# Rinoahu/pangenome

Hardware: AMD Instinct MI355X
Metric: Gbp/s k-mer->rdBG build at k=27; bit-exact region table vs numba ref (higher is better)
Workload: dtype u8; 1 GPU; C3: 100 x 5 Mbp variants (0.1% SNP, 0.01% indel), two alternating batches of the same population (genomes 0-99, 100-199); k=27, strands=-c 2 (dBG both strands), bases_per_gpu=500000568, fasta_bytes_per_gpu=508334450, parallelism=single GPU

## Files before the change

### pangenome_amd/csrc/pg_abi.hip

```cpp
#include <chrono>
#include <cstring>
#include <string>

#include "../../include/pangenome.h"
#include "pg_internal.h"
#include "pg_text.h"

struct pg_ctx {
  pg::Ctx c;
};

static thread_local std::string g_err;

template <class F>
static int guard(F&& f) {
  try {
    f();
    return PG_OK;
  } catch (const pg::Error& e) {
    g_err = e.what();
    return e.code;
  } catch (const std::bad_alloc&) {
    g_err = "out of host memory";
    return PG_ENOMEM;
// ... 45 lines not shown
    PG_HIP(hipStreamCreateWithFlags(&x->c.stream3, hipStreamNonBlocking));
    {
      int lo = 0, hi = 0;
      PG_HIP(hipDeviceGetStreamPriorityRange(&lo, &hi));
      PG_HIP(hipStreamCreateWithPriority(&x->c.stream_hi, hipStreamNonBlocking, hi));
    }
    for (auto& e : x->c.ev) PG_HIP(hipEventCreateWithFlags(&e, hipEventDisableTiming));
    for (auto& e : x->c.cev) PG_HIP(hipEventCreateWithFlags(&e, hipEventDisableTiming));
    PG_HIP(hipEventCreateWithFlags(&x->c.rec_ev, hipEventDisableTiming));
    PG_HIP(hipEventCreateWithFlags(&x->c.ext_ev, hipEventDisableTiming));
    PG_HIP(hipDeviceGetAttribute(&x->c.n_cu, hipDeviceAttributeMultiprocessorCount, device));
    *out = x;
  });
}

void pg_destroy(pg_ctx* x) {
  if (!x) return;
  pg::Ctx& c = x->c;
  (void)hipSetDevice(c.device);
  (void)hipStreamSynchronize(c.stream);
  pg::DevBuf* bufs[] = {&c.fasta_own, &c.span_sum, &c.span_start, &c.n_sel, &c.rec_start, &c.rec_len,
                        &c.rec_hdr, &c.rec_ptr, &c.rec_flag, &c.cls, &c.p2, &c.e16, &c.scratch, &c.table, &c.ovf, &c.flags,
                        &c.recA_key, &c.recA_mw, &c.ctrA, &c.recS_key[0], &c.recS_key[1], &c.recS_mw[0],
                        &c.recS_mw[1], &c.ctrS, &c.snapA, &c.rseg, &c.k5_ctr, &c.tile_sched, &c.tile_desc, &c.k3_queue,
                        &c.k3_hint, &c.part_cnt, &c.tile_cnt, &c.tile_off, &c.occ, &c.edge_tab, &c.pair_tab,
                        &c.edge_out, &c.edge_exp, &c.lab_tab, &c.lab_list, &c.rows_buf, &c.xyz_off,
                        &c.text_buf, &c.clu_text, &c.mk_mat, &c.fr_tab, &c.fr_spec, &c.fr_grp, &c.fr_text,
                        &c.cmp_shared, &c.cmp_curve, &c.nj_dist, &c.rg_nodes, &c.rg_links, &c.rg_paths, &c.rg_steps, &c.rg_text,
                        &c.rs_tab, &c.rs_blob, &c.preload,
                        &c.dump_cnt};
  for (auto* b : bufs) b->release();
  pg::pool_destroy(c);
  c.stage_pin.release();
  c.rec_pack.release();
  c.h_pin.release();
  c.h_out.release();
  c.tile_pin.release();
  for (auto& b : c.dump_pin) b.release();
  c.t0.destroy();
  c.t1.destroy();
  c.t6.destroy();
  c.t_rs.destroy();
  c.t_nj.destroy();
  for (auto& t : c.t_bt) t.destroy();
  for (auto& e : c.ev)
    if (e) (void)hipEventDestroy(e);
  for (auto e : c.cev)
// ... 1365 lines not shown
```

### pangenome_amd/csrc/pg_dbg.hip

```cpp
#include <algorithm>
#include <type_traits>
#include <cstdio>
#include <cstdlib>
#include <cstring>

#include <rocprim/rocprim.hpp>

#include "pg_internal.h"

#ifndef PG_EXP_BITS
#define PG_EXP_BITS 0
#endif

namespace pg {

#ifdef PG_DEBUG_BOUNDS
__device__ unsigned long long g_dbg[16 + 16 * 4 * 5];
__device__ __forceinline__ bool pg_bok(bool ok, unsigned code, long long a, long long b) {
  if (!ok) {
    const unsigned slot = code % 16;
    const unsigned long long i = atomicAdd(&g_dbg[slot], 1ull);
    if (i < 4) {
      unsigned long long* e = g_dbg + 16 + (slot * 4 + i) * 5;
      e[0] = code; e[1] = (unsigned long long)a; e[2] = (unsigned long long)b; e[3] = blockIdx.x; e[4] = threadIdx.x;
// ... 427 lines not shown
  }
  return covered;
}

struct Stage {
  long long qt, a0, hi, plo, phi, ra0, rend;
};
__device__ __forceinline__ void ref_span(Stage& g, int k, long long rfs, long long rfn) {
  g.plo = g.qt - 1 - DRIFT > 0 ? g.qt - 1 - DRIFT : 0;
  g.phi = g.qt + TILE + k + 1 + DRIFT < rfn ? g.qt + TILE + k + 1 + DRIFT : rfn;
  g.ra0 = (rfs + g.plo) & ~15ll;
  g.rend = rfs + g.phi;
}
__device__ __forceinline__ Stage stage_of(const TileDesc& td, int k, bool dedup, long long rfs, long long rfn) {
  Stage g;
  g.qt = (long long)td.stripe * TILE;
  const long long lo = td.rs + (g.qt >= 2 ? g.qt - 2 : 0);
  g.hi = td.rs + (g.qt + TILE + k + 2 < td.rn ? g.qt + TILE + k + 2 : td.rn);
  g.a0 = lo & ~15ll;
  g.plo = g.phi = g.ra0 = g.rend = 0;
  if (dedup) ref_span(g, k, rfs, rfn);
  return g;
}

__host__ __device__ __forceinline__ void xcd_chunk(uint64_t ntiles, uint32_t b0, uint32_t b1, uint32_t bt, uint64_t x,
                                                   uint64_t& t, uint64_t& te) {
  const uint64_t xs = ntiles * x / 8, xl = ntiles * (x + 1) / 8 - xs;
  t = xs + xl * b0 / bt;
  te = xs + xl * b1 / bt;
}

#ifdef PG_COVER_LEGACY
__global__ void __launch_bounds__(CBLOCK)
k_cover(const uint8_t* __restrict__ cls, const TileDesc* __restrict__ descs, WorkItem* __restrict__ queue,
        unsigned long long* __restrict__ qcount, unsigned long long qcap, int k, int ref, long long rfs,
        long long rfn, int ref2, long long r2s, long long r2n, int* __restrict__ hints, int nrec,
        uint64_t ngroups, uint32_t b0, uint32_t b1, uint32_t bt) {
  __shared__ __attribute__((aligned(16))) uint8_t s_cls[QM][SPAN + 16];
  __shared__ __attribute__((aligned(16))) uint8_t s_ref[2][RSPAN];
  __shared__ unsigned s_best[QM][2][NANCH];
  __shared__ uint32_t s_scan[CBLOCK / 64];
  __shared__ unsigned long long s_qbase;
  __shared__ MemGeo s_geo[QM];
  __shared__ Drifts s_dr[QM][2];
  uint64_t g, ge;
  xcd_chunk(ngroups, b0, b1, bt, blockIdx.x & 7, g, ge);
// ... 390 lines not shown
          const int s = 4 * (3 * ri + j);
          const uint32_t nz = ((w0 >> s) & 15u) | ((w1 >> s) & 15u) << 4 | ((w2 >> s) & 15u) << 8;
          covered |= ((rel >= lo) & (rel <= hi)) ? map_cover(nz, sh, k) : 0u;
        }
      }
    }
    cov[m] = covered;
    const bool work = ((live >> m) & 1u) && q0 <= last && covered != (1u << IW) - 1u;
    wmask |= (uint32_t)work << m;
    nwk += work ? 1u : 0u;
  }
  uint32_t nwork;
  uint32_t pos = block_excl_scan<CBLOCK>(nwk, s_scan, nwork);
  const unsigned sub = blockIdx.x % NQ;
  if (t == 0) s_qbase = nwork ? atomicAdd(qcount + QSTRIDE * sub, (unsigned long long)nwork) : 0ull;
  __syncthreads();
#pragma unroll
  for (int m = 0; m < QM; ++m)
    if ((wmask >> m) & 1u) queue[sub * qcap + s_qbase + pos++] = WorkItem{mrs[m], mrn[m] - k, q0, cov[m], 0u};
}

#endif

struct TriGeo {
  int ibhi, lo, hi, lo1, hi1;
};

constexpr int RPADW = 4;
constexpr int RSTAGEW = (RSPAN + 15) / 16 + 2;
constexpr int RDW = (RPADW + RSTAGEW + 16 + 3) / 4 * 4;
constexpr int LW = 7;
static_assert(IW * 4 == 64 && CBLOCK == 64 * QM, "a lane owns 4 segments; a wave owns a member");
#ifndef PG_HWIN2P
#define PG_HWIN2P 56
#endif
constexpr int HWIN2P = PG_HWIN2P;
constexpr int NAP_DEFAULT = 4;
template <int NAP>
constexpr int astep_p() { return (TILE - ALEN - 16) / (NAP - 1); }

template <int NAP>
struct Drifts2 {
  int n;
  int U[NAP], lo[NAP], hi[NAP];
  int d[NAP];
};
__device__ __forceinline__ uint32_t p2_word(const uint32_t* p2, long long i, uint64_t n_p2) {
  return (i >= 0 && (uint64_t)i < n_p2) ? p2[i] : 0u;
}
// ... 77 lines not shown
  }
  auto take = [&](auto W) {
    constexpr int w = decltype(W)::value;
#pragma unroll
    for (int i = 0; i < 8; ++i) out[i] = raw[w + i];
  };
  switch (__builtin_amdgcn_readfirstlane(idx & 3)) {
    case 0: take(std::integral_constant<int, 0>{}); break;
    case 1: take(std::integral_constant<int, 1>{}); break;
    case 2: take(std::integral_constant<int, 2>{}); break;
    default: take(std::integral_constant<int, 3>{}); break;
  }
}
__device__ __forceinline__ uint32_t even_bits(uint32_t x) {
  x = (x | (x >> 1)) & 0x33333333u;
  x = (x | (x >> 2)) & 0x0F0F0F0Fu;
  x = (x | (x >> 4)) & 0x00FF00FFu;
  return (x | (x >> 8)) & 0x0000FFFFu;
}

template <int NAP>
__global__ void __launch_bounds__(CBLOCK, 8)
k_cover_p(const uint32_t* __restrict__ p2, const uint8_t* __restrict__ e16, uint64_t n_p2,
          const uint8_t* __restrict__ cls_dbg, const TileDesc* __restrict__ descs, WorkItem* __restrict__ queue, unsigned long long* __restrict__ qcount,
          unsigned long long qcap, int k, int ref, long long rfs, long long rfn, int ref2, long long r2s,
          long long r2n, int* __restrict__ hints, int nrec, uint64_t ngroups, uint32_t b0, uint32_t b1, uint32_t bt) {
  static_assert(NAP >= 2 && QM * NAP + QM * 2 * NAP <= CBLOCK, "anchor loads and triple geometry: one thread each");
  constexpr int ASTEPP = astep_p<NAP>();
  __shared__ __attribute__((aligned(16))) uint32_t s_ref[2][RDW];
  __shared__ uint32_t s_anc[QM][NAP][2];
  __shared__ unsigned s_best[QM][2][NAP];
  __shared__ uint32_t s_scan[CBLOCK / 64];
  __shared__ unsigned long long s_qbase;
  __shared__ Drifts2<NAP> s_dr[QM][2];
  __shared__ TriGeo s_tri[QM * 2 * NAP];
  __shared__ uint32_t s_rexc;
  uint64_t g, ge;
  xcd_chunk(ngroups, b0, b1, bt, blockIdx.x & 7, g, ge);
  g += blockIdx.x >> 3;
  if (g >= ge) return;
  const int t = (int)threadIdx.x;
  const long long qt = (long long)descs[QM * g].stripe * TILE;
  RefGeo rg[2];
  long long rd0[2];
  int rnw[2];
#pragma unroll
  for (int ri = 0; ri < 2; ++ri) {
    const long long s = ri ? r2s : rfs, n = ri ? r2n : rfn;
    rg[ri].plo = qt - 1 - DRIFT > 0 ? qt - 1 - DRIFT : 0;
    rg[ri].phi = qt + TILE + k + 1 + DRIFT < n ? qt + TILE + k + 1 + DRIFT : n;
    rg[ri].rfn = n;
    rd0[ri] = (s + rg[ri].plo) >> 4;
    rnw[ri] = (int)(((s + rg[ri].phi + 15) >> 4) - rd0[ri]);
    rg[ri].rbase = 16 * RPADW + s - 16 * rd0[ri];
  }
  long long mrs[QM], mrn[QM];
  uint32_t dm0 = 0, dm1 = 0, live = 0;
#pragma unroll
  for (int m = 0; m < QM; ++m) {
    const TileDesc td = descs[QM * g + m];
    mrs[m] = td.rs;
    mrn[m] = td.rn;
    const bool d0 = td.r >= 0 && ref >= 0 && ref != td.r;
    live |= (uint32_t)(td.r >= 0) << m;
    dm0 |= (uint32_t)d0 << m;
    dm1 |= (uint32_t)(d0 && ref2 >= 0 && ref2 != td.r) << m;
  }
  const int mw = __builtin_amdgcn_readfirstlane(t >> 6), lw = t & 63;
  uint32_t M[LW], eex = 0;
  {
    long long rsm = mrs[0];
#pragma unroll
    for (int y = 1; y < QM; ++y) if (mw == y) rsm = mrs[y];
    const long long wb = ((rsm + qt - 1) >> 4) + 4 * lw, a = wb & ~3ll;
    const bool on = (dm0 >> mw) & 1u;
#pragma unroll
    for (int i = 0; i < LW; ++i) M[i] = on ? p2_word(p2, wb + i, n_p2) : 0u;
#pragma unroll
    for (int i = 0; i < 3; ++i)
      if (on && a + 4 * i >= 0 && (uint64_t)(a + 4 * i + 4) <= n_p2 + 16)
        eex |= *reinterpret_cast<const uint32_t*>(e16 + a + 4 * i);
  }
  if (t == 0) s_rexc = 0u;
  if (t < QM * NAP) {
    const int m = t / NAP, ai = t % NAP;
    long long rs = mrs[0];
#pragma unroll
    for (int y = 1; y < QM; ++y) rs = m == y ? mrs[y] : rs;
    const long long ga = rs + qt + 8 + (long long)ai * ASTEPP, x = ga >> 4;
    const uint32_t sb = 2u * (uint32_t)(ga & 15);
    uint32_t P0 = 0, P1 = 0, P2 = 0;
    if ((dm0 >> m) & 1u) { P0 = p2_word(p2, x, n_p2); P1 = p2_word(p2, x + 1, n_p2); P2 = p2_word(p2, x + 2, n_p2); }
    s_anc[m][ai][0] = __builtin_amdgcn_alignbit(P1, P0, sb);
    s_anc[m][ai][1] = __builtin_amdgcn_alignbit(P2, P1, sb);
  } else if (t >= CBLOCK - QM * 2 * NAP) {
    const int x = t - (CBLOCK - QM * 2 * NAP), m = x / (2 * NAP), ri = (x / NAP) & 1, ai = x % NAP;
    (&s_best[0][0][0])[x] = ~0u;
    TriGeo G{0, 0, -1, 0, -1};
    if ((((ri ? dm1 : dm0) >> m) & 1u)) {
      const TileDesc td = descs[QM * g + m];
      const int hh = hints[(size_t)(blockIdx.x & 7) * 2 * nrec + (ri ? nrec : 0) + td.r];
      const int h = hh < 0 ? DRIFT : hh;
      const RefGeo& R = ri ? rg[1] : rg[0];
      const long long a = qt + 8 + (long long)ai * ASTEPP;
      G.ibhi = (int)(R.rbase + a + DRIFT);
      G.lo = max(G.ibhi - 2 * DRIFT, (int)(R.rbase + R.plo));
      G.hi = a + ALEN > td.rn ? -1 : min(G.ibhi, (int)(R.rbase + R.phi) - ALEN);
      G.lo1 = max(G.lo, G.ibhi - (h + HWIN2P));
      G.hi1 = min(G.hi, G.ibhi - (h - HWIN2P));
    }
    s_tri[x] = G;
  }
  cover_barrier();
  {
    static_assert(RSTAGEW <= 2 * CBLOCK, "two words per thread and reference");
    uint32_t v[2][2], ex = 0;
#pragma unroll
    for (int ri = 0; ri < 2; ++ri) {
      const int nw = (ri ? dm1 != 0 : dm0 != 0) ? rnw[ri] : 0;
#pragma unroll
      for (int h = 0; h < 2; ++h) {
        const int i = t + h * CBLOCK;
        v[ri][h] = i < nw ? p2_word(p2, rd0[ri] + i, n_p2) : 0u;
        if (i < nw && PG_BOK(rd0[ri] + i >= 0 && (uint64_t)(rd0[ri] + i) < n_p2, 12, rd0[ri] + i, n_p2) &&
            e16[rd0[ri] + i])
          ex |= 1u << ri;
      }
    }
#pragma unroll
    for (int ri = 0; ri < 2; ++ri)
#pragma unroll
      for (int h = 0; h < 2; ++h)
        if (t + h * CBLOCK < rnw[ri] && PG_BOK(RPADW + t + h * CBLOCK < RDW, 13, rnw[ri], t))
          s_ref[ri][RPADW + t + h * CBLOCK] = v[ri][h];
    if (ex) atomicOr(&s_rexc, ex);
  }
  cover_barrier();
  {
    const uint32_t rexc = s_rexc;
    if (rexc & 1u) dm0 = dm1 = 0u;
    if (rexc & 2u) dm1 = 0u;
  }
  if (dm0) cover_search_p(s_anc, s_ref, s_tri, s_best, dm0, dm1);
  if (t < QM * 2 * NAP) {
    const int m = t / (2 * NAP), ri = (t / NAP) & 1, ai = t % NAP;
    if ((((ri ? dm1 : dm0) >> m) & 1u)) {
      const unsigned* B = s_best[m][ri];
      const unsigned b = B[ai];
      auto first = [&](int j) {
        if (B[j] == ~0u) return false;
        for (int i = 0; i < j; ++i)
          if ((B[i] & 0xFFFFu) == (B[j] & 0xFFFFu)) return false;
        return true;
      };
      int slot = 0;
      for (int j = 0; j < ai; ++j) slot += first(j) ? 1 : 0;
      const bool keep = first(ai);
      bool last = b != ~0u;
      for (int j = ai + 1; j < NAP; ++j) last &= B[j] == ~0u;
      long long rs = mrs[0];
#pragma unroll
      for (int y = 1; y < QM; ++y) rs = m == y ? mrs[y] : rs;
      const int r = descs[QM * g + m].r;
      (void)PG_BOK(r >= 0 && r < nrec, 52, (long long)r, (long long)nrec);
      if (last) hints[(size_t)(blockIdx.x & 7) * 2 * nrec + (ri ? nrec : 0) + r] = (int)(b & 0xFFFFu);
      Drifts2<NAP>& D = s_dr[m][ri];
      if (keep) {
        const RefGeo R = ri ? rg[1] : rg[0];
        const long long pos16 = 16 * ((rs + qt - 1) >> 4) - rs;
        const int d = (int)(b & 0xFFFFu) - DRIFT;
        const long long pl = R.plo + 1 > 1 ? R.plo + 1 : 1;
        const long long ph = R.rfn - k - IW < R.phi - IW - k ? R.rfn - k - IW : R.phi - IW - k;
        const long long lo = pl + d - qt, hi = ph + d - qt;
        D.U[slot] = (int)(R.rbase + pos16 - d);
        D.lo[slot] = (int)(lo < -(1ll << 30) ? -(1ll << 30) : lo);
        D.hi[slot] = (int)(hi > (1ll << 30) ? (1ll << 30) : hi);
        D.d[slot] = d;
      }
      if (ai == NAP - 1) D.n = slot + (keep ? 1 : 0);
    }
  }
  cover_barrier();
  const int m = __builtin_amdgcn_readfirstlane(t >> 6), l = t & 63;
  long long rs = mrs[0], rn = mrn[0];
#pragma unroll
  for (int y = 1; y < QM; ++y) if (m == y) { rs = mrs[y]; rn = mrn[y]; }
  const long long last = rn - k;
  uint32_t covS[4] = {0u, 0u, 0u, 0u};
  bool mex = false;
  if ((dm0 >> m) & 1u) {
    const long long p0 = rs + qt - 1, wb = (p0 >> 4) + 4 * l;
    const int sh2 = 2 * (int)(p0 & 15);
    (void)PG_BOK(wb + LW <= (long long)n_p2 + 4 || wb > (long long)n_p2, 11, wb, n_p2);
    (void)wb;
    mex = eex != 0u;
    const int L = k + 2;
    const int P = L >= 16 ? 16 : L >= 8 ? 8 : L >= 4 ? 4 : 2;
    const uint32_t rsh = 2u * (uint32_t)(L - P);
#pragma unroll
    for (int ri = 0; ri < 2; ++ri) {
      if (ri && !((dm1 >> m) & 1u)) break;
      const int nd = __builtin_amdgcn_readfirstlane(s_dr[m][ri].n);
#pragma unroll 1
      for (int j = 0; j < nd; ++j) {
        const int U = __builtin_amdgcn_readfirstlane(s_dr[m][ri].U[j]);
        const int lo = __builtin_amdgcn_readfirstlane(s_dr[m][ri].lo[j]);
        const int hi = __builtin_amdgcn_readfirstlane(s_dr[m][ri].hi[j]);
        int iw = (U >> 4) + 4 * l;
        if (iw < 0 || iw + 12 > RDW) iw &= 3;
        if (!PG_BOK(iw >= 0 && iw + 12 <= RDW, 14, iw, U)) iw = 0;
        uint32_t raw[12];
        {
          const uint4* r16 = reinterpret_cast<const uint4*>(s_ref[ri]);
#pragma unroll
          for (int q = 0; q < 3; ++q) {
            uint4 v = r16[(iw >> 2) + q];
            asm volatile("" : "+v"(v.x), "+v"(v.y), "+v"(v.z), "+v"(v.w));
            raw[4 * q] = v.x; raw[4 * q + 1] = v.y; raw[4 * q + 2] = v.z; raw[4 * q + 3] = v.w;
// ... 32 lines not shown
          covS[s] |= (rel >= lo && rel <= hi) ? ~S & 0x55555555u : 0u;
#ifdef PG_DEBUG_BOUNDS
          {
            const long long q0 = qt + rel;
            const int dd = __builtin_amdgcn_readfirstlane(s_dr[m][ri].d[j]);
            const long long fs = ri ? r2s : rfs;
            const uint32_t cvd = (rel >= lo && rel <= hi && q0 > 0 && q0 + IW <= last) ? (~S & 0x55555555u) : 0u;
            for (int i = 0; i < 16; ++i)
              if ((cvd >> (2 * i)) & 1u) {
                const long long q = q0 + i;
                bool eq = true;
                for (int x = -1; x <= k; ++x) eq &= cls_dbg[rs + q + x] == cls_dbg[fs + q - dd + x];
                (void)pg_bok(eq, 31, (long long)q, (long long)dd);
              }
          }
#endif
        }
      }
    }
  }
  uint32_t nwk = 0, wmask = 0, cov[4];
#pragma unroll
  for (int s = 0; s < 4; ++s) {
    const long long q0 = qt + 64 * l + 16 * s;
    const bool interior = q0 > 0 && q0 + IW <= last;
    cov[s] = interior && !mex ? even_bits(covS[s]) : 0u;
    const bool work = ((live >> m) & 1u) && q0 <= last && cov[s] != (1u << IW) - 1u;
    wmask |= (uint32_t)work << s;
    nwk += work ? 1u : 0u;
  }
  uint32_t nwork;
  uint32_t pos = block_excl_scan<CBLOCK>(nwk, s_scan, nwork);
  const unsigned sub = blockIdx.x % NQ;
  if (t == 0) {
    s_qbase = nwork ? atomicAdd(qcount + QSTRIDE * sub, (unsigned long long)nwork) : 0ull;
    (void)PG_BOK(nwork <= QM * CBLOCK && s_qbase + nwork <= qcap, 42, (long long)nwork, (long long)s_qbase);
  }
  cover_barrier();
#pragma unroll
  for (int s = 0; s < 4; ++s)
    if ((wmask >> s) & 1u) {
      if (PG_BOK(s_qbase + pos < qcap && rs >= 0 && qt + 64 * l + 16 * s <= rn, 15, s_qbase + pos, rs))
        queue[sub * qcap + s_qbase + pos] = WorkItem{rs, rn - k, qt + 64 * l + 16 * s, cov[s], 0u};
      ++pos;
    }
}

template <typename... A>
static void launch_cover_p(int na, dim3 grid, hipStream_t s, A... a) {
  switch (na) {
    case 3: hipLaunchKernelGGL(k_cover_p<3>, grid, dim3(CBLOCK), 0, s, a...); break;
    case 4: hipLaunchKernelGGL(k_cover_p<4>, grid, dim3(CBLOCK), 0, s, a...); break;
    case 5: hipLaunchKernelGGL(k_cover_p<5>, grid, dim3(CBLOCK), 0, s, a...); break;
    case 6: hipLaunchKernelGGL(k_cover_p<6>, grid, dim3(CBLOCK), 0, s, a...); break;
    default: hipLaunchKernelGGL(k_cover_p<8>, grid, dim3(CBLOCK), 0, s, a...); break;
  }
}

#ifdef PG_DEBUG_BOUNDS
__global__ void k_dbg_counters(const unsigned long long* __restrict__ qcount, unsigned long long lim, unsigned code,
                               unsigned chunk) {
  const unsigned sub = threadIdx.x;
  if (sub < NQ) {
    const unsigned long long v = qcount[QSTRIDE * sub];
    (void)pg_bok(v <= lim, code, (long long)v, (long long)(chunk * 1000 + sub));
  }
// ... 687 lines not shown
    b += __shfl_down(b, o, 64);
    m += __shfl_down(m, o, 64);
  }
  if ((threadIdx.x & 63) == 0) {
    s_red[0][threadIdx.x >> 6] = a;
    s_red[1][threadIdx.x >> 6] = b;
    s_red[2][threadIdx.x >> 6] = m;
  }
  __syncthreads();
  if (threadIdx.x == 0) {
    unsigned long long sa = 0, sb = 0, sm = 0;
    for (int w = 0; w < RB_T / 64; ++w) { sa += s_red[0][w]; sb += s_red[1][w]; sm += s_red[2][w]; }
    unsigned long long* o = R.ctr + (uint64_t)blockIdx.x * RB_CTR;
    o[0] = sa;
    o[1] = sb;
    if constexpr (KEYS) o[2] = s_mcur;
    else o[2] = sm;
  }
}

constexpr uint32_t LEAD = 4;
__global__ void k_tiles(const uint32_t* __restrict__ sched, uint32_t nj, uint32_t lead_stripes, uint32_t lead_off,
                        const long long* __restrict__ rec_start, const long long* __restrict__ rec_len,
                        TileDesc* __restrict__ out, uint64_t ngroups) {
  const uint32_t* off = sched;
  const uint32_t* nf = sched + nj + 1;
  const uint32_t* ord = nf + nj;
  for (uint64_t t = blockIdx.x * (uint64_t)blockDim.x + threadIdx.x; t < ngroups * QM;
       t += (uint64_t)gridDim.x * blockDim.x) {
    const uint64_t g = t / QM;
    const uint32_t m = (uint32_t)(t % QM);
    uint32_t lo = 0, hi = nj;
    while (hi - lo > 1) {
      const uint32_t mid = (lo + hi) >> 1;
      if (off[mid] <= g) lo = mid; else hi = mid;
    }
    uint32_t i = (uint32_t)(g - off[lo]);
    const bool lead = lo < lead_stripes;
    int r = -1, stripe;
    if (lead && i == 0) {
      stripe = (int)lo;
      if (m == 0) r = (int)ord[0];
    } else {
      if (lead) --i;
      stripe = (int)(lo - lead_off);
      const uint32_t f = i * QM + m;
      if (f < nf[lo]) r = (int)ord[1 + f];
    }
    out[t] = r >= 0 ? TileDesc{rec_start[r], rec_len[r], r, stripe, 0} : TileDesc{0, 0, -1, stripe, 0};
  }
}

constexpr int EXE = 8;
__global__ void __launch_bounds__(256) k_export_dbg(TableView T, uint64_t nw, uint64_t ntot, int k,
                                                   unsigned long long* __restrict__ keys,
                                                   unsigned short* __restrict__ masks, uint64_t cap,
                                                   unsigned long long* __restrict__ counter) {
  __shared__ uint32_t s_scan[4];
  __shared__ unsigned long long s_base;
  for (uint64_t c0 = blockIdx.x * (uint64_t)(256 * EXE); c0 < ntot; c0 += (uint64_t)gridDim.x * 256 * EXE) {
    uint32_t m[EXE];
    uint32_t cnt = 0;
#pragma unroll
    for (int e = 0; e < EXE; ++e) {
      const uint64_t i = c0 + (uint64_t)threadIdx.x * EXE + e;
      m[e] = i < ntot ? entry_mask(T, nw, i) : 0u;
      cnt += ((m[e] & PRES_A) ? 1u : 0u) + ((m[e] & PRES_B) ? 1u : 0u);
    }
    uint32_t tot;
    const uint32_t pre = block_excl_scan<256>(cnt, s_scan, tot);
    if (threadIdx.x == 0) s_base = tot ? atomicAdd(counter, (unsigned long long)tot) : 0ull;
    __syncthreads();
// ... 211 lines not shown
  const uint32_t lead_off = follow ? 0u : LEAD;
  const uint32_t nj = nt.empty() ? 0u : (uint32_t)(follow ? nt[0].first : lead_s + LEAD);
  const size_t skip = follow ? 0 : 1;
  std::vector<uint32_t> sched(2 * nj + 2 + nt.size());
  uint64_t total = 0;
  size_t live = nt.size();
  for (uint32_t j = 0; j < nj; ++j) {
    sched[j] = (uint32_t)total;
    uint64_t cnt = j < lead_s ? 1 : 0, nfol = 0;
    if (j >= lead_off) {
      const uint64_t jf = j - lead_off;
      while (live && nt[live - 1].first <= jf) --live;
      nfol = live > skip ? live - skip : 0;
      cnt += (nfol + QM - 1) / QM;
    }
    sched[nj + 1 + j] = (uint32_t)nfol;
    total += cnt;
  }
  sched[nj] = (uint32_t)total;
  if (follow) sched[2 * nj + 1] = 0u;
  for (size_t i = 0; i < nt.size(); ++i) sched[2 * nj + 1 + (follow ? 1 : 0) + i] = (uint32_t)nt[i].second;
  if (total * QM >= (1ull << 32)) throw Error(-22, "make_tiles: too many tiles");
  c.tile_desc.reserve(sizeof(TileDesc) * (QM * total + 1));
  if (total) {
    c.tile_pin.reserve(4 * sched.size());
    c.tile_sched.reserve(4 * sched.size());
    std::memcpy(c.tile_pin.p, sched.data(), 4 * sched.size());
    PG_HIP(hipMemcpyAsync(c.tile_sched.p, c.tile_pin.p, 4 * sched.size(), hipMemcpyHostToDevice, st));
    hipLaunchKernelGGL(k_tiles, dim3(grid_for(QM * total, 256, 2048)), dim3(256), 0, st,
                       c.tile_sched.as<uint32_t>(), nj, (uint32_t)lead_s, lead_off, c.rec_start.as<long long>(),
                       c.rec_len.as<long long>(), c.tile_desc.as<TileDesc>(), total);
    PG_HIP(hipGetLastError());
  }
  if (follow) {
    c.tile_sig_len.clear();
  } else {
    c.tile_sig_len = c.h_rec_len;
    c.tile_sig_flag = flag;
    c.tile_k = c.k;
  }
  c.n_tiles = total;
  return total;
}

static BinOut stageA_begin(Ctx& c, uint64_t cap, FillList& fl, bool reset = true) {
  if (reset) {
    c.capA = cap;
    c.recA_key.reserve(8 * NREG * cap);
    c.recA_mw.reserve(4 * NREG * cap);
    c.ctrA.reserve(8 * CSTRIDE * NREG);
    c.flags.reserve(4 * N_FLAGS + 16 * MCHK);
    fl.add(c.ctrA.p, 8 * CSTRIDE * NREG);
    fl.add(c.flags.p, 4 * N_FLAGS + 16 * MCHK);
  }
// ... 269 lines not shown
  if (!c.n_records) return;
  hipLaunchKernelGGL(k_short_emit, dim3(grid_for(c.n_records, IBLOCK, 1024)), dim3(IBLOCK), 0, s, packed_cls(c),
                     c.rec_start.as<long long>(), c.rec_len.as<long long>(), c.rec_flag.as<uint8_t>(), c.n_records,
                     c.k, shift, rc0, c.tv, O);
  PG_HIP(hipGetLastError());
}

enum { SA_WHOLE = 0, SA_FIRST = 1, SA_MORE = 2, SA_TAIL = 3, SA_FIRST_TAIL = 4, SA_MORE_TAIL = 5 };
static void enqueue_stageA(Ctx& c, uint64_t cap, uint64_t ntiles, int rc0, int extra_empty, int part = SA_WHOLE,
                           bool join = true) {
  const uint64_t shift = pow5(c.k - 1);
  hipStream_t s0 = c.stream, s1 = c.stream2;
  FillList fl;
  const bool begin = part == SA_WHOLE || part == SA_FIRST || part == SA_FIRST_TAIL;
  const bool tail = part == SA_WHOLE || part == SA_TAIL || part == SA_FIRST_TAIL || part == SA_MORE_TAIL;
  const BinOut O = stageA_begin(c, cap, fl, begin);
  if (part == SA_TAIL) ntiles = 0;
#ifdef PG_COVER_LEGACY
  if (c.k3_cover == 1 || c.k3_cover == 2) ensure_cls(c);
#endif
#ifdef PG_DEBUG_BOUNDS
  ensure_cls(c);
#endif
  const uint8_t* cls = c.cls.as<uint8_t>();
  const PackedCls pc = packed_cls(c);
  const dim3 b(IBLOCK);
  int nch = ntiles >= (uint64_t)K3_CHUNKS * K3_CHUNK_MIN ? K3_CHUNKS : 1;
  if (c.k3_chunks > 0) nch = std::min(6, c.k3_chunks);
  if (!ntiles) nch = 0;
  const uint32_t tailw = c.k3_tail ? (uint32_t)c.k3_tail : 10u;
  const uint32_t headw = c.k3_head ? (uint32_t)c.k3_head : 16u;
  uint32_t cb[8] = {};
  for (int i = 1; i <= nch; ++i) cb[i] = cb[i - 1] + (i == nch ? tailw : i == 1 ? headw : 16u);
  const uint32_t cbt = nch ? cb[nch] : 1u;
  uint64_t gc[8] = {}, qoff[8] = {}, qcapc[8] = {}, items = 0;
  for (int i = 0; i < nch; ++i) {
    for (int x = 0; x < 8; ++x) {
      uint64_t t, te;
      xcd_chunk(ntiles, cb[i], cb[i + 1], cbt, (uint64_t)x, t, te);
      gc[i] = std::max<uint64_t>(gc[i], 8 * (te - t));
    }
    qcapc[i] = (gc[i] + NQ - 1) / NQ * (QM * CBLOCK);
    qoff[i] = items;
    items += NQ * qcapc[i];
  }
  const size_t qbytes = sizeof(WorkItem) * items, cbytes = 8 * QSTRIDE * NQ;
  if (nch) {
    c.k3_queue.reserve(qbytes + cbytes * nch);
    fl.add(c.k3_queue.as<uint8_t>() + qbytes, cbytes * nch);
    fl.add(c.k3_hint.p, 16 * 4 * (c.n_records + 1), 0xFFFFFFFFu);
  }
  const bool side = part == SA_WHOLE;
  if (side) {
    fl.launch(s1);
    PG_HIP(hipEventRecord(c.ev[0], s1));
    PG_HIP(hipStreamWaitEvent(s0, c.ev[0], 0));
  }
  c.t1.init();
  c.t1.start(s0);
  if (!side) fl.launch(s0);
#ifdef PG_DEBUG_BOUNDS
  for (int i = 0; i < nch; ++i)
    hipLaunchKernelGGL(k_dbg_counters, dim3(1), dim3(64), 0, s0,
                       reinterpret_cast<const unsigned long long*>(c.k3_queue.as<uint8_t>() + qbytes) + (cbytes / 8) * i,
                       0ull, 41u, (unsigned)i);
#endif
  const unsigned wgrid = (unsigned)c.n_cu * (c.k3_wblk & 15 ? c.k3_wblk & 15 : K3_WBLK);
  const unsigned wgrid_last = c.k3_wblk >> 4 ? (unsigned)c.n_cu * (c.k3_wblk >> 4) : wgrid;
  auto* q = c.k3_queue.as<WorkItem>();
  auto* qn = reinterpret_cast<unsigned long long*>(c.k3_queue.as<uint8_t>() + qbytes);
  const long long rfs = c.k3_ref >= 0 ? c.h_rec_start[c.k3_ref] : 0, rfn = c.k3_ref >= 0 ? c.h_rec_len[c.k3_ref] : 0;
  const long long r2s = c.k3_ref2 >= 0 ? c.h_rec_start[c.k3_ref2] : 0;
  const long long r2n = c.k3_ref2 >= 0 ? c.h_rec_len[c.k3_ref2] : 0;
  const TileDesc* td = c.tile_desc.as<TileDesc>();
  bool short_done = false;
  if (!side) {
    PG_HIP(hipEventRecord(c.ev[0], s0));
    PG_HIP(hipStreamWaitEvent(s1, c.ev[0], 0));
  }
  for (int i = 0; i < nch; ++i) {
    auto* qi = q + qoff[i];
    auto* qni = qn + (cbytes / 8) * i;
#ifdef PG_COVER_LEGACY
    if (gc[i] && c.k3_cover == 1)
      hipLaunchKernelGGL(k_cover, dim3((unsigned)gc[i]), dim3(CBLOCK), 0, s0, cls, td, qi, qni, (unsigned long long)qcapc[i],
                         c.k, c.k3_ref, rfs, rfn, c.k3_ref2, r2s, r2n, c.k3_hint.as<int>(), (int)c.n_records, ntiles,
                         cb[i], cb[i + 1], cbt);
    else if (gc[i] && c.k3_cover == 2)
      hipLaunchKernelGGL(k_cover_q, dim3((unsigned)gc[i]), dim3(CBLOCK), 0, s0, cls, (uint64_t)c.cls.cap, td, qi, qni,
                         (unsigned long long)qcapc[i], c.k, c.k3_ref, rfs, rfn, c.k3_ref2, r2s, r2n,
                         c.k3_hint.as<int>(), (int)c.n_records, ntiles, cb[i], cb[i + 1], cbt);
    else
#endif
    if (gc[i])
      launch_cover_p(c.k3_anchors ? c.k3_anchors : NAP_DEFAULT, dim3((unsigned)gc[i]), s0, c.p2.as<uint32_t>(),
                     c.e16.as<uint8_t>(), (uint64_t)(c.p2.cap / 4), cls, td, qi, qni, (unsigned long long)qcapc[i], c.k,
                     c.k3_ref, rfs, rfn, c.k3_ref2, r2s, r2n, c.k3_hint.as<int>(), (int)c.n_records, ntiles,
                     cb[i], cb[i + 1], cbt);
    PG_HIP(hipGetLastError());
#ifdef PG_DEBUG_BOUNDS
    for (int j = 0; j < nch; ++j)
      hipLaunchKernelGGL(k_dbg_counters, dim3(1), dim3(64), 0, s0, qn + (cbytes / 8) * j,
                         j <= i ? (unsigned long long)qcapc[j] : 0ull, j <= i ? 43u : 44u, (unsigned)(i * 10 + j));
#endif
    hipStream_t ws = s1;
    if (nch > 1 && i + 1 == nch) {
      ws = s0;
      if (tail) {
        launch_short(c, s1, rc0, shift, O);
        short_done = true;
      }
    } else {
      PG_HIP(hipEventRecord(c.ev[1 + i], s0));
      PG_HIP(hipStreamWaitEvent(s1, c.ev[1 + i], 0));
    }
    const uint64_t mi = std::min<uint64_t>(NQ * qcapc[i], c.windows_fw / IW + c.n_records + 1);
    const unsigned gw = nch > 1 ? (i + 1 == nch ? wgrid_last : wgrid) : grid_for(mi, IBLOCK, 16384);
    const bool halves = c.k3_emit != 1;
    auto* kw = rc0 ? (halves ? k_emit_work<true, 2> : k_emit_work<true, 1>)
                   : (halves ? k_emit_work<false, 2> : k_emit_work<false, 1>);
    hipLaunchKernelGGL(kw, dim3(gw), b, 0, ws, pc, qi, qni, (unsigned long long)qcapc[i], c.k, shift, c.tv, O);
// ... 581 lines not shown
```

### pangenome_amd/csrc/pg_internal.h

```cpp
#pragma once
#include <hip/hip_runtime.h>

#include <algorithm>
#include <atomic>
#include <chrono>
#include <cstdint>
#include <cstdlib>
#include <cstring>
#include <stdexcept>
#include <string>
#include <functional>
#include <vector>

#include "pg_common.h"

namespace pg {

struct Error : std::runtime_error {
  int code;
  Error(int c, const std::string& m) : std::runtime_error(m), code(c) {}
};

#define PG_HIP(x)                                                                       \
  do {                                                                                  \
// ... 197 lines not shown
  DevBuf k5_ctr;
  uint64_t rseg_cap = 0, rseg_nseg = 0;
  std::vector<uint64_t> rseg_cnt;
  uint64_t n_records_a = 0;
  double u_ratio = 0, r_ratio = 0;

  DevBuf tile_sched;
  PinBuf tile_pin;
  uint64_t n_tiles = 0;
  int tile_k = 0;
  int k3_ref = -1;
  int k3_ref2 = -1;
  DevBuf part_cnt;
  uint64_t part_counts[64] = {};
  uint64_t part_sums[64] = {};
  uint64_t merge_sum = 0, merge_rows = 0;
  uint64_t work_items = 0;
  uint64_t part_total = 0;
  int part_nparts = 0;
  uint64_t part_gen = ~0ull;
  uint64_t build_gen = 0;
  DevBuf k3_hint;
  DevBuf tile_desc;
  DevBuf k3_queue;
  std::vector<int64_t> tile_sig_len;
  std::vector<uint8_t> tile_sig_flag;

  DevBuf tile_cnt, tile_off;
  DevBuf occ;
  DevBuf edge_tab, pair_tab;
  DevBuf edge_out;
  DevBuf edge_exp;
  uint64_t edge_cap = 0, pair_cap = 0, n_edges = 0;
  bool edges_ready = false;
  DevBuf lab_tab;
  uint64_t lab_cap = 0;
  DevBuf lab_list;
  uint64_t n_labels = 0;
  DevBuf rows_buf;
  uint64_t n_rows = 0;
  bool rows_ready = false;
  DevBuf xyz_off;
  uint64_t xyz_total = 0;
  bool xyz_sized = false;
  DevBuf text_buf;
  DevBuf clu_text;
// ... 388 lines not shown
```

Before: 443.8 Gbp/s.

## Precompute per-group cover geometry in k_tiles and hoist reference loads in k_cover_p

k_tiles now also writes a 16-byte-aligned GroupGeo record per tile group, holding the stripe offset, member/dedup bitmasks, per-member word bases, shifts and relative bounds, and per-reference span parameters. k_cover_p reads this record instead of recomputing it from TileDesc entries and 64-bit reference arithmetic. The per-XCD chunk bounds are now computed on the host and passed as a kernel argument, and the reference-word loads are issued before the first barrier rather than after it. The aim is to cut scalar and divergent setup work and to overlap the global loads in the cover kernel. The cost is an extra device buffer, a heavier k_tiles kernel, and values clamped to 30 bits, which relies on relative offsets staying within that range.

Result: no change. 452.8 Gbp/s, median of 6 (+2.0%).

```diff
diff --git a/pangenome_amd/csrc/pg_abi.hip b/pangenome_amd/csrc/pg_abi.hip
--- a/pangenome_amd/csrc/pg_abi.hip
+++ b/pangenome_amd/csrc/pg_abi.hip
@@ -91,7 +91,7 @@
   pg::DevBuf* bufs[] = {&c.fasta_own, &c.span_sum, &c.span_start, &c.n_sel, &c.rec_start, &c.rec_len,
                         &c.rec_hdr, &c.rec_ptr, &c.rec_flag, &c.cls, &c.p2, &c.e16, &c.scratch, &c.table, &c.ovf, &c.flags,
                         &c.recA_key, &c.recA_mw, &c.ctrA, &c.recS_key[0], &c.recS_key[1], &c.recS_mw[0],
-                        &c.recS_mw[1], &c.ctrS, &c.snapA, &c.rseg, &c.k5_ctr, &c.tile_sched, &c.tile_desc, &c.k3_queue,
+                        &c.recS_mw[1], &c.ctrS, &c.snapA, &c.rseg, &c.k5_ctr, &c.tile_sched, &c.tile_desc, &c.tile_geo, &c.k3_queue,
                         &c.k3_hint, &c.part_cnt, &c.tile_cnt, &c.tile_off, &c.occ, &c.edge_tab, &c.pair_tab,
                         &c.edge_out, &c.edge_exp, &c.lab_tab, &c.lab_list, &c.rows_buf, &c.xyz_off,
                         &c.text_buf, &c.clu_text, &c.mk_mat, &c.fr_tab, &c.fr_spec, &c.fr_grp, &c.fr_text,
diff --git a/pangenome_amd/csrc/pg_dbg.hip b/pangenome_amd/csrc/pg_dbg.hip
--- a/pangenome_amd/csrc/pg_dbg.hip
+++ b/pangenome_amd/csrc/pg_dbg.hip
@@ -473,6 +473,10 @@
   if (dedup) ref_span(g, k, rfs, rfn);
   return g;
 }
+
+struct TriGeo {
+  int ibhi, lo, hi, lo1, hi1;
+};
 
 __host__ __device__ __forceinline__ void xcd_chunk(uint64_t ntiles, uint32_t b0, uint32_t b1, uint32_t bt, uint64_t x,
                                                    uint64_t& t, uint64_t& te) {
@@ -909,9 +913,41 @@
 
 #endif
 
-struct TriGeo {
-  int ibhi, lo, hi, lo1, hi1;
+struct RefSpan {
+  long long rd0;
+  int rnw;
+  int ph;
+  int ibhi0, lomin, himax;
+  int pl;
 };
+struct MemberGeo {
+  long long rs, last;
+  long long wb;
+  int r;
+  int sh2;
+  int lastrel;
+  int arel;
+  int U0[2];
+};
+struct alignas(16) GroupGeo {
+  long long qt;
+  uint32_t bits;
+  uint32_t pad;
+  RefSpan ref[2];
+  MemberGeo mem[QM];
+};
+static_assert(QM <= 8 && sizeof(RefSpan) == 32 && sizeof(MemberGeo) == 48 && sizeof(GroupGeo) == 16 + 64 + 48 * QM &&
+                  sizeof(GroupGeo) % 16 == 0,
+              "wide aligned loads of a header, a reference or a member");
+struct HintGeo {
+  int r, U0, pl, ph;
+};
+struct XcdBounds {
+  uint32_t g0[8], ge[8];
+};
+__host__ __device__ __forceinline__ int clamp30(long long v) {
+  return (int)(v < -(1ll << 30) ? -(1ll << 30) : v > (1ll << 30) ? (1ll << 30) : v);
+}
 
 constexpr int RPADW = 4;
 constexpr int RSTAGEW = (RSPAN + 15) / 16 + 2;
@@ -1035,9 +1071,11 @@
 template <int NAP>
 __global__ void __launch_bounds__(CBLOCK, 8)
 k_cover_p(const uint32_t* __restrict__ p2, const uint8_t* __restrict__ e16, uint64_t n_p2,
-          const uint8_t* __restrict__ cls_dbg, const TileDesc* __restrict__ descs, WorkItem* __restrict__ queue, unsigned long long* __restrict__ qcount,
-          unsigned long long qcap, int k, int ref, long long rfs, long long rfn, int ref2, long long r2s,
-          long long r2n, int* __restrict__ hints, int nrec, uint64_t ngroups, uint32_t b0, uint32_t b1, uint32_t bt) {
+#ifdef PG_DEBUG_BOUNDS
+          const uint8_t* __restrict__ cls_dbg, long long rfs, long long r2s,
+#endif
+          const GroupGeo* __restrict__ geo, WorkItem* __restrict__ queue, unsigned long long* __restrict__ qcount,
+          unsigned long long qcap, int k, int* __restrict__ hints, int nrec, XcdBounds xb) {
   static_assert(NAP >= 2 && QM * NAP + QM * 2 * NAP <= CBLOCK, "anchor loads and triple geometry: one thread each");
   constexpr int ASTEPP = astep_p<NAP>();
   __shared__ __attribute__((aligned(16))) uint32_t s_ref[2][RDW];
@@ -1047,60 +1085,47 @@
   __shared__ unsigned long long s_qbase;
   __shared__ Drifts2<NAP> s_dr[QM][2];
   __shared__ TriGeo s_tri[QM * 2 * NAP];
+  __shared__ HintGeo s_hg[QM * 2 * NAP];
   __shared__ uint32_t s_rexc;
-  uint64_t g, ge;
-  xcd_chunk(ngroups, b0, b1, bt, blockIdx.x & 7, g, ge);
-  g += blockIdx.x >> 3;
-  if (g >= ge) return;
+  const uint32_t xcd = blockIdx.x & 7;
+  const uint32_t g = xb.g0[xcd] + (blockIdx.x >> 3);
+  if (g >= xb.ge[xcd]) return;
   const int t = (int)threadIdx.x;
-  const long long qt = (long long)descs[QM * g].stripe * TILE;
-  RefGeo rg[2];
-  long long rd0[2];
-  int rnw[2];
+  const GroupGeo& G = geo[g];
+  const int mw = __builtin_amdgcn_readfirstlane(t >> 6), lw = t & 63;
+  const MemberGeo& me = G.mem[mw];
+  const long long qt = G.qt;
+  const uint32_t live = G.bits & 0xFFu;
+  uint32_t dm0 = (G.bits >> 8) & 0xFFu, dm1 = (G.bits >> 16) & 0xFFu;
+  uint32_t M[LW], eex[3];
+  {
+    const long long wb = me.wb + 4 * lw, a = wb & ~3ll;
+    const bool on = (dm0 >> mw) & 1u;
+#pragma unroll
+    for (int i = 0; i < LW; ++i) M[i] = on ? p2_word(p2, wb + i, n_p2) : 0u;
+#pragma unroll
+    for (int i = 0; i < 3; ++i)
+      eex[i] = on && a + 4 * i >= 0 && (uint64_t)(a + 4 * i + 4) <= n_p2 + 16
+                   ? *reinterpret_cast<const uint32_t*>(e16 + a + 4 * i) : 0u;
+  }
+  static_assert(RSTAGEW <= 2 * CBLOCK, "two words per thread and reference");
+  uint32_t rv[2][2], rx[2][2];
 #pragma unroll
   for (int ri = 0; ri < 2; ++ri) {
-    const long long s = ri ? r2s : rfs, n = ri ? r2n : rfn;
-    rg[ri].plo = qt - 1 - DRIFT > 0 ? qt - 1 - DRIFT : 0;
-    rg[ri].phi = qt + TILE + k + 1 + DRIFT < n ? qt + TILE + k + 1 + DRIFT : n;
-    rg[ri].rfn = n;
-    rd0[ri] = (s + rg[ri].plo) >> 4;
-    rnw[ri] = (int)(((s + rg[ri].phi + 15) >> 4) - rd0[ri]);
-    rg[ri].rbase = 16 * RPADW + s - 16 * rd0[ri];
-  }
-  long long mrs[QM], mrn[QM];
-  uint32_t dm0 = 0, dm1 = 0, live = 0;
-#pragma unroll
-  for (int m = 0; m < QM; ++m) {
-    const TileDesc td = descs[QM * g + m];
-    mrs[m] = td.rs;
-    mrn[m] = td.rn;
-    const bool d0 = td.r >= 0 && ref >= 0 && ref != td.r;
-    live |= (uint32_t)(td.r >= 0) << m;
-    dm0 |= (uint32_t)d0 << m;
-    dm1 |= (uint32_t)(d0 && ref2 >= 0 && ref2 != td.r) << m;
-  }
-  const int mw = __builtin_amdgcn_readfirstlane(t >> 6), lw = t & 63;
-  uint32_t M[LW], eex = 0;
-  {
-    long long rsm = mrs[0];
-#pragma unroll
-    for (int y = 1; y < QM; ++y) if (mw == y) rsm = mrs[y];
-    const long long wb = ((rsm + qt - 1) >> 4) + 4 * lw, a = wb & ~3ll;
-    const bool on = (dm0 >> mw) & 1u;
-#pragma unroll
-    for (int i = 0; i < LW; ++i) M[i] = on ? p2_word(p2, wb + i, n_p2) : 0u;
-#pragma unroll
-    for (int i = 0; i < 3; ++i)
-      if (on && a + 4 * i >= 0 && (uint64_t)(a + 4 * i + 4) <= n_p2 + 16)
-        eex |= *reinterpret_cast<const uint32_t*>(e16 + a + 4 * i);
+    const long long rd0 = G.ref[ri].rd0;
+    const int nw = (ri ? dm1 != 0 : dm0 != 0) ? G.ref[ri].rnw : 0;
+#pragma unroll
+    for (int h = 0; h < 2; ++h) {
+      const int i = t + h * CBLOCK;
+      rv[ri][h] = i < nw ? p2_word(p2, rd0 + i, n_p2) : 0u;
+      rx[ri][h] = i < nw && PG_BOK(rd0 + i >= 0 && (uint64_t)(rd0 + i) < n_p2, 12, rd0 + i, n_p2) ? e16[rd0 + i] : 0u;
+    }
   }
   if (t == 0) s_rexc = 0u;
   if (t < QM * NAP) {
     const int m = t / NAP, ai = t % NAP;
-    long long rs = mrs[0];
-#pragma unroll
-    for (int y = 1; y < QM; ++y) rs = m == y ? mrs[y] : rs;
-    const long long ga = rs + qt + 8 + (long long)ai * ASTEPP, x = ga >> 4;
+    const int ga = (G.mem[m].sh2 >> 1) + 9 + ai * ASTEPP;
+    const long long x = G.mem[m].wb + (ga >> 4);
     const uint32_t sb = 2u * (uint32_t)(ga & 15);
     uint32_t P0 = 0, P1 = 0, P2 = 0;
     if ((dm0 >> m) & 1u) { P0 = p2_word(p2, x, n_p2); P1 = p2_word(p2, x + 1, n_p2); P2 = p2_word(p2, x + 2, n_p2); }
@@ -1109,43 +1134,32 @@
   } else if (t >= CBLOCK - QM * 2 * NAP) {
     const int x = t - (CBLOCK - QM * 2 * NAP), m = x / (2 * NAP), ri = (x / NAP) & 1, ai = x % NAP;
     (&s_best[0][0][0])[x] = ~0u;
-    TriGeo G{0, 0, -1, 0, -1};
+    const MemberGeo& mg = G.mem[m];
+    const RefSpan& R = G.ref[ri];
+    const int r = mg.r;
+    s_hg[x] = HintGeo{r, mg.U0[ri], R.pl, R.ph};
+    TriGeo T{0, 0, -1, 0, -1};
     if ((((ri ? dm1 : dm0) >> m) & 1u)) {
-      const TileDesc td = descs[QM * g + m];
-      const int hh = hints[(size_t)(blockIdx.x & 7) * 2 * nrec + (ri ? nrec : 0) + td.r];
+      const int hh = hints[(size_t)xcd * 2 * nrec + (ri ? nrec : 0) + r];
       const int h = hh < 0 ? DRIFT : hh;
-      const RefGeo& R = ri ? rg[1] : rg[0];
-      const long long a = qt + 8 + (long long)ai * ASTEPP;
-      G.ibhi = (int)(R.rbase + a + DRIFT);
-      G.lo = max(G.ibhi - 2 * DRIFT, (int)(R.rbase + R.plo));
-      G.hi = a + ALEN > td.rn ? -1 : min(G.ibhi, (int)(R.rbase + R.phi) - ALEN);
-      G.lo1 = max(G.lo, G.ibhi - (h + HWIN2P));
-      G.hi1 = min(G.hi, G.ibhi - (h - HWIN2P));
-    }
-    s_tri[x] = G;
+      T.ibhi = R.ibhi0 + ai * ASTEPP;
+      T.lo = max(T.ibhi - 2 * DRIFT, R.lomin);
+      T.hi = ai * ASTEPP > mg.arel ? -1 : min(T.ibhi, R.himax);
+      T.lo1 = max(T.lo, T.ibhi - (h + HWIN2P));
+      T.hi1 = min(T.hi, T.ibhi - (h - HWIN2P));
+    }
+    s_tri[x] = T;
   }
   cover_barrier();
   {
-    static_assert(RSTAGEW <= 2 * CBLOCK, "two words per thread and reference");
-    uint32_t v[2][2], ex = 0;
-#pragma unroll
-    for (int ri = 0; ri < 2; ++ri) {
-      const int nw = (ri ? dm1 != 0 : dm0 != 0) ? rnw[ri] : 0;
-#pragma unroll
-      for (int h = 0; h < 2; ++h) {
-        const int i = t + h * CBLOCK;
-        v[ri][h] = i < nw ? p2_word(p2, rd0[ri] + i, n_p2) : 0u;
-        if (i < nw && PG_BOK(rd0[ri] + i >= 0 && (uint64_t)(rd0[ri] + i) < n_p2, 12, rd0[ri] + i, n_p2) &&
-            e16[rd0[ri] + i])
-          ex |= 1u << ri;
-      }
-    }
+    const int rnw[2] = {G.ref[0].rnw, G.ref[1].rnw};
 #pragma unroll
     for (int ri = 0; ri < 2; ++ri)
 #pragma unroll
       for (int h = 0; h < 2; ++h)
         if (t + h * CBLOCK < rnw[ri] && PG_BOK(RPADW + t + h * CBLOCK < RDW, 13, rnw[ri], t))
-          s_ref[ri][RPADW + t + h * CBLOCK] = v[ri][h];
+          s_ref[ri][RPADW + t + h * CBLOCK] = rv[ri][h];
+    const uint32_t ex = ((rx[0][0] | rx[0][1]) ? 1u : 0u) | ((rx[1][0] | rx[1][1]) ? 2u : 0u);
     if (ex) atomicOr(&s_rexc, ex);
   }
   cover_barrier();
@@ -1171,42 +1185,30 @@
       const bool keep = first(ai);
       bool last = b != ~0u;
       for (int j = ai + 1; j < NAP; ++j) last &= B[j] == ~0u;
-      long long rs = mrs[0];
-#pragma unroll
-      for (int y = 1; y < QM; ++y) rs = m == y ? mrs[y] : rs;
-      const int r = descs[QM * g + m].r;
-      (void)PG_BOK(r >= 0 && r < nrec, 52, (long long)r, (long long)nrec);
-      if (last) hints[(size_t)(blockIdx.x & 7) * 2 * nrec + (ri ? nrec : 0) + r] = (int)(b & 0xFFFFu);
+      const HintGeo hg = s_hg[t];
+      (void)PG_BOK(hg.r >= 0 && hg.r < nrec, 52, (long long)hg.r, (long long)nrec);
+      if (last) hints[(size_t)xcd * 2 * nrec + (ri ? nrec : 0) + hg.r] = (int)(b & 0xFFFFu);
       Drifts2<NAP>& D = s_dr[m][ri];
       if (keep) {
-        const RefGeo R = ri ? rg[1] : rg[0];
-        const long long pos16 = 16 * ((rs + qt - 1) >> 4) - rs;
         const int d = (int)(b & 0xFFFFu) - DRIFT;
-        const long long pl = R.plo + 1 > 1 ? R.plo + 1 : 1;
-        const long long ph = R.rfn - k - IW < R.phi - IW - k ? R.rfn - k - IW : R.phi - IW - k;
-        const long long lo = pl + d - qt, hi = ph + d - qt;
-        D.U[slot] = (int)(R.rbase + pos16 - d);
-        D.lo[slot] = (int)(lo < -(1ll << 30) ? -(1ll << 30) : lo);
-        D.hi[slot] = (int)(hi > (1ll << 30) ? (1ll << 30) : hi);
+        D.U[slot] = hg.U0 - d;
+        D.lo[slot] = hg.pl + d;
+        D.hi[slot] = hg.ph + d;
         D.d[slot] = d;
       }
       if (ai == NAP - 1) D.n = slot + (keep ? 1 : 0);
     }
   }
   cover_barrier();
-  const int m = __builtin_amdgcn_readfirstlane(t >> 6), l = t & 63;
-  long long rs = mrs[0], rn = mrn[0];
-#pragma unroll
-  for (int y = 1; y < QM; ++y) if (m == y) { rs = mrs[y]; rn = mrn[y]; }
-  const long long last = rn - k;
+  const int m = mw, l = lw;
+  const long long rs = me.rs, last = me.last;
+  const int lastrel = me.lastrel;
   uint32_t covS[4] = {0u, 0u, 0u, 0u};
   bool mex = false;
   if ((dm0 >> m) & 1u) {
-    const long long p0 = rs + qt - 1, wb = (p0 >> 4) + 4 * l;
-    const int sh2 = 2 * (int)(p0 & 15);
-    (void)PG_BOK(wb + LW <= (long long)n_p2 + 4 || wb > (long long)n_p2, 11, wb, n_p2);
-    (void)wb;
-    mex = eex != 0u;
+    const int sh2 = me.sh2;
+    (void)PG_BOK(me.wb + 4 * l + LW <= (long long)n_p2 + 4 || me.wb + 4 * l > (long long)n_p2, 11, me.wb + 4 * l, n_p2);
+    mex = (eex[0] | eex[1] | eex[2]) != 0u;
     const int L = k + 2;
     const int P = L >= 16 ? 16 : L >= 8 ? 8 : L >= 4 ? 4 : 2;
     const uint32_t rsh = 2u * (uint32_t)(L - P);
@@ -1285,10 +1287,10 @@
   uint32_t nwk = 0, wmask = 0, cov[4];
 #pragma unroll
   for (int s = 0; s < 4; ++s) {
-    const long long q0 = qt + 64 * l + 16 * s;
-    const bool interior = q0 > 0 && q0 + IW <= last;
+    const int rel = 64 * l + 16 * s;
+    const bool interior = (rel > 0 || qt > 0) && rel + IW <= lastrel;
     cov[s] = interior && !mex ? even_bits(covS[s]) : 0u;
-    const bool work = ((live >> m) & 1u) && q0 <= last && cov[s] != (1u << IW) - 1u;
+    const bool work = ((live >> m) & 1u) && rel <= lastrel && cov[s] != (1u << IW) - 1u;
     wmask |= (uint32_t)work << s;
     nwk += work ? 1u : 0u;
   }
@@ -1303,8 +1305,8 @@
 #pragma unroll
   for (int s = 0; s < 4; ++s)
     if ((wmask >> s) & 1u) {
-      if (PG_BOK(s_qbase + pos < qcap && rs >= 0 && qt + 64 * l + 16 * s <= rn, 15, s_qbase + pos, rs))
-        queue[sub * qcap + s_qbase + pos] = WorkItem{rs, rn - k, qt + 64 * l + 16 * s, cov[s], 0u};
+      if (PG_BOK(s_qbase + pos < qcap && rs >= 0 && qt + 64 * l + 16 * s <= last + k, 15, s_qbase + pos, rs))
+        queue[sub * qcap + s_qbase + pos] = WorkItem{rs, last, qt + 64 * l + 16 * s, cov[s], 0u};
       ++pos;
     }
 }
@@ -2038,7 +2040,8 @@
 constexpr uint32_t LEAD = 4;
 __global__ void k_tiles(const uint32_t* __restrict__ sched, uint32_t nj, uint32_t lead_stripes, uint32_t lead_off,
                         const long long* __restrict__ rec_start, const long long* __restrict__ rec_len,
-                        TileDesc* __restrict__ out, uint64_t ngroups) {
+                        TileDesc* __restrict__ out, GroupGeo* __restrict__ geo, uint64_t ngroups, int k, int ref,
+                        long long rfs, long long rfn, int ref2, long long r2s, long long r2n) {
   const uint32_t* off = sched;
   const uint32_t* nf = sched + nj + 1;
   const uint32_t* ord = nf + nj;
@@ -2052,18 +2055,61 @@
       if (off[mid] <= g) lo = mid; else hi = mid;
     }
     uint32_t i = (uint32_t)(g - off[lo]);
-    const bool lead = lo < lead_stripes;
-    int r = -1, stripe;
-    if (lead && i == 0) {
-      stripe = (int)lo;
-      if (m == 0) r = (int)ord[0];
-    } else {
-      if (lead) --i;
-      stripe = (int)(lo - lead_off);
-      const uint32_t f = i * QM + m;
-      if (f < nf[lo]) r = (int)ord[1 + f];
-    }
-    out[t] = r >= 0 ? TileDesc{rec_start[r], rec_len[r], r, stripe, 0} : TileDesc{0, 0, -1, stripe, 0};
+    const bool lead = lo < lead_stripes, alone = lead && i == 0;
+    if (lead && !alone) --i;
+    const int stripe = alone ? (int)lo : (int)(lo - lead_off);
+    auto rec_of = [&](uint32_t mm) {
+      if (alone) return mm == 0 ? (int)ord[0] : -1;
+      const uint32_t f = i * QM + mm;
+      return f < nf[lo] ? (int)ord[1 + f] : -1;
+    };
+    const int r = rec_of(m);
+    const long long rs = r >= 0 ? rec_start[r] : 0, rn = r >= 0 ? rec_len[r] : 0;
+    out[t] = TileDesc{rs, rn, r, stripe, 0};
+    const long long qt = (long long)stripe * TILE;
+    GroupGeo& G = geo[g];
+    MemberGeo mg;
+    mg.rs = rs;
+    mg.last = rn - k;
+    mg.wb = (rs + qt - 1) >> 4;
+    mg.r = r;
+    mg.sh2 = 2 * (int)((rs + qt - 1) & 15);
+    mg.lastrel = clamp30(rn - k - qt);
+    mg.arel = clamp30(rn - qt - 8 - ALEN);
+    const long long pos16 = 16 * mg.wb - rs;
+#pragma unroll
+    for (int ri = 0; ri < 2; ++ri) {
+      const long long s = ri ? r2s : rfs, n = ri ? r2n : rfn;
+      const long long plo = qt - 1 - DRIFT > 0 ? qt - 1 - DRIFT : 0;
+      const long long phi = qt + TILE + k + 1 + DRIFT < n ? qt + TILE + k + 1 + DRIFT : n;
+      const long long rd0 = (s + plo) >> 4, rbase = 16 * RPADW + s - 16 * rd0;
+      mg.U0[ri] = clamp30(rbase + pos16);
+      if (m == 0) {
+        RefSpan R;
+        R.rd0 = rd0;
+        R.rnw = clamp30(((s + phi + 15) >> 4) - rd0);
+        R.ph = clamp30((n < phi ? n : phi) - k - IW - qt);
+        R.ibhi0 = clamp30(rbase + qt + 8 + DRIFT);
+        R.lomin = clamp30(rbase + plo);
+        R.himax = clamp30(rbase + phi) - ALEN;
+        R.pl = clamp30((plo + 1 > 1 ? plo + 1 : 1) - qt);
+        G.ref[ri] = R;
+      }
+    }
+    G.mem[m] = mg;
+    if (m == 0) {
+      uint32_t bits = 0;
+#pragma unroll
+      for (uint32_t mm = 0; mm < QM; ++mm) {
+        const int rr = rec_of(mm);
+        const bool d0 = rr >= 0 && ref >= 0 && ref != rr;
+        bits |= (uint32_t)(rr >= 0) << mm | (uint32_t)d0 << (8 + mm) |
+                (uint32_t)(d0 && ref2 >= 0 && ref2 != rr) << (16 + mm);
+      }
+      G.qt = qt;
+      G.bits = bits;
+      G.pad = 0;
+    }
   }
 }
 
@@ -2321,14 +2367,18 @@
   for (size_t i = 0; i < nt.size(); ++i) sched[2 * nj + 1 + (follow ? 1 : 0) + i] = (uint32_t)nt[i].second;
   if (total * QM >= (1ull << 32)) throw Error(-22, "make_tiles: too many tiles");
   c.tile_desc.reserve(sizeof(TileDesc) * (QM * total + 1));
+  c.tile_geo.reserve(sizeof(GroupGeo) * (total + 1));
   if (total) {
     c.tile_pin.reserve(4 * sched.size());
     c.tile_sched.reserve(4 * sched.size());
     std::memcpy(c.tile_pin.p, sched.data(), 4 * sched.size());
     PG_HIP(hipMemcpyAsync(c.tile_sched.p, c.tile_pin.p, 4 * sched.size(), hipMemcpyHostToDevice, st));
+    const int r1 = c.k3_ref, r2 = c.k3_ref2;
     hipLaunchKernelGGL(k_tiles, dim3(grid_for(QM * total, 256, 2048)), dim3(256), 0, st,
                        c.tile_sched.as<uint32_t>(), nj, (uint32_t)lead_s, lead_off, c.rec_start.as<long long>(),
-                       c.rec_len.as<long long>(), c.tile_desc.as<TileDesc>(), total);
+                       c.rec_len.as<long long>(), c.tile_desc.as<TileDesc>(), c.tile_geo.as<GroupGeo>(), total, c.k,
+                       r1, (long long)(r1 >= 0 ? c.h_rec_start[r1] : 0), (long long)(r1 >= 0 ? c.h_rec_len[r1] : 0), r2,
+                       (long long)(r2 >= 0 ? c.h_rec_start[r2] : 0), (long long)(r2 >= 0 ? c.h_rec_len[r2] : 0));
     PG_HIP(hipGetLastError());
   }
   if (follow) {
@@ -2644,7 +2694,9 @@
 #ifdef PG_DEBUG_BOUNDS
   ensure_cls(c);
 #endif
+#if defined(PG_COVER_LEGACY) || defined(PG_DEBUG_BOUNDS)
   const uint8_t* cls = c.cls.as<uint8_t>();
+#endif
   const PackedCls pc = packed_cls(c);
   const dim3 b(IBLOCK);
   int nch = ntiles >= (uint64_t)K3_CHUNKS * K3_CHUNK_MIN ? K3_CHUNKS : 1;
@@ -2656,11 +2708,14 @@
   for (int i = 1; i <= nch; ++i) cb[i] = cb[i - 1] + (i == nch ? tailw : i == 1 ? headw : 16u);
   const uint32_t cbt = nch ? cb[nch] : 1u;
   uint64_t gc[8] = {}, qoff[8] = {}, qcapc[8] = {}, items = 0;
+  XcdBounds xb[8] = {};
   for (int i = 0; i < nch; ++i) {
     for (int x = 0; x < 8; ++x) {
       uint64_t t, te;
       xcd_chunk(ntiles, cb[i], cb[i + 1], cbt, (uint64_t)x, t, te);
       gc[i] = std::max<uint64_t>(gc[i], 8 * (te - t));
+      xb[i].g0[x] = (uint32_t)t;
+      xb[i].ge[x] = (uint32_t)te;
     }
     qcapc[i] = (gc[i] + NQ - 1) / NQ * (QM * CBLOCK);
     qoff[i] = items;
@@ -2691,10 +2746,15 @@
   const unsigned wgrid_last = c.k3_wblk >> 4 ? (unsigned)c.n_cu * (c.k3_wblk >> 4) : wgrid;
   auto* q = c.k3_queue.as<WorkItem>();
   auto* qn = reinterpret_cast<unsigned long long*>(c.k3_queue.as<uint8_t>() + qbytes);
-  const long long rfs = c.k3_ref >= 0 ? c.h_rec_start[c.k3_ref] : 0, rfn = c.k3_ref >= 0 ? c.h_rec_len[c.k3_ref] : 0;
+#if defined(PG_COVER_LEGACY) || defined(PG_DEBUG_BOUNDS)
+  const long long rfs = c.k3_ref >= 0 ? c.h_rec_start[c.k3_ref] : 0;
   const long long r2s = c.k3_ref2 >= 0 ? c.h_rec_start[c.k3_ref2] : 0;
+#endif
+#ifdef PG_COVER_LEGACY
+  const long long rfn = c.k3_ref >= 0 ? c.h_rec_len[c.k3_ref] : 0;
   const long long r2n = c.k3_ref2 >= 0 ? c.h_rec_len[c.k3_ref2] : 0;
   const TileDesc* td = c.tile_desc.as<TileDesc>();
+#endif
   bool short_done = false;
   if (!side) {
     PG_HIP(hipEventRecord(c.ev[0], s0));
@@ -2716,9 +2776,12 @@
 #endif
     if (gc[i])
       launch_cover_p(c.k3_anchors ? c.k3_anchors : NAP_DEFAULT, dim3((unsigned)gc[i]), s0, c.p2.as<uint32_t>(),
-                     c.e16.as<uint8_t>(), (uint64_t)(c.p2.cap / 4), cls, td, qi, qni, (unsigned long long)qcapc[i], c.k,
-                     c.k3_ref, rfs, rfn, c.k3_ref2, r2s, r2n, c.k3_hint.as<int>(), (int)c.n_records, ntiles,
-                     cb[i], cb[i + 1], cbt);
+                     c.e16.as<uint8_t>(), (uint64_t)(c.p2.cap / 4),
+#ifdef PG_DEBUG_BOUNDS
+                     cls, (long long)rfs, (long long)r2s,
+#endif
+                     c.tile_geo.as<GroupGeo>(), qi, qni, (unsigned long long)qcapc[i], c.k, c.k3_hint.as<int>(),
+                     (int)c.n_records, xb[i]);
     PG_HIP(hipGetLastError());
 #ifdef PG_DEBUG_BOUNDS
     for (int j = 0; j < nch; ++j)
diff --git a/pangenome_amd/csrc/pg_internal.h b/pangenome_amd/csrc/pg_internal.h
--- a/pangenome_amd/csrc/pg_internal.h
+++ b/pangenome_amd/csrc/pg_internal.h
@@ -243,6 +243,7 @@
   uint64_t build_gen = 0;
   DevBuf k3_hint;
   DevBuf tile_desc;
+  DevBuf tile_geo;
   DevBuf k3_queue;
   std::vector<int64_t> tile_sig_len;
   std::vector<uint8_t> tile_sig_flag;
```
